# ChrisDud0257/GSASR

Hardware: AMD Instinct MI355X
Metric: HR Mpixels/sec fwd+bwd (x4, 1 Gaussian/LR px); achieved HBM GB/s vs roofline (higher is better)
Workload: dtype f32; 1 GPU; config2: 256x256 LR -> x4 (1024^2 HR), 65536 Gaussians, fwd+bwd; H=1024, W=1024, gaussians=65536, cutoff_k_box=336, launch=eager (faster than hipgraph replay: 67.6 vs 75.3 us/step), forward_subtile_px=8, parallelism=single

## Files before the change

### gsasr_amd/csrc/splat_common.h

```cpp
#ifndef GSASR_SPLAT_COMMON_H
#define GSASR_SPLAT_COMMON_H
#include <hip/hip_runtime.h>

#include <atomic>
#include <cmath>
#include <cstdint>
#include <cstdio>
#include <cstdlib>
#include <cstring>
#include <mutex>
#include <vector>

#include "gsasr_splat.h"

namespace gsasr_detail {

int fail(int code, const char *msg);
int hip_fail(hipError_t e, const char *where);
const char *last_error_message();
struct KernelChoice { unsigned flags; int list_cap; };
KernelChoice registered_choice(const gsasr_dims *d);
float default_cutoff();
void store_default_cutoff(float tau);

// ... 476 lines not shown
    if (cutoff != 0.f) return cutoff;
    const double tau = std::log((double)(s > 1 ? s : 1) / (double)GSASR_SPLAT_DEFAULT_EPS);
    return (float)(tau < 16.0 ? 16.0 : tau > (double)GSASR_SPLAT_EXACT_CUTOFF ? (double)GSASR_SPLAT_EXACT_CUTOFF : tau);
}

inline bool batch_uniform(const gsasr_dims *d, int &h, int &w)
{
    h = w = 0;
    if (d->batch <= 1) return false;
    for (int b = 1; b < d->batch; ++b)
        if (d->sample_hw[2 * b] != d->sample_hw[0] || d->sample_hw[2 * b + 1] != d->sample_hw[1]) return false;
    h = d->sample_hw[0];
    w = d->sample_hw[1];
    return true;
}

inline Params make_params(const gsasr_dims *d, const Layout &L, const gsasr_view *vw = nullptr)
{
    Params P;
    const gsasr_dims pd = policy_dims(d, vw);
    const bool bviews = vw && d->batch > 1;
    double scale_w = vw ? (double)vw->full_w : (double)d->w, scale_h = vw ? (double)vw->full_h : (double)d->h;
    double full_wmin = scale_w, full_hmin = scale_h;
    if (bviews) {
        for (int b = 1; b < d->batch; ++b) {
            scale_w = std::fmax(scale_w, (double)vw[b].full_w);
            scale_h = std::fmax(scale_h, (double)vw[b].full_h);
            full_wmin = std::fmin(full_wmin, (double)vw[b].full_w);
            full_hmin = std::fmin(full_hmin, (double)vw[b].full_h);
        }
    }
    P.s = d->s; P.h = d->h; P.w = d->w; P.row0 = d->row0; P.row1 = d->row1;
    P.bounded = d->dmax >= 0.f;
    P.dmax = P.bounded ? d->dmax : INFINITY;
    const float tau = resolve_cutoff(d->cutoff, d->s);
    P.kcut = tau > 0.f ? (float)(std::sqrt(2.0 * (double)tau) * (1.0 + 1e-6)) : 0.f;
    P.adapt_cells = P.adapt_cells4 = 0.f;
    P.adapt_ring = 0;
    P.count_words = (int)(L.count_bytes / 4);
    P.ext_groups = L.ext_groups;
    P.dead_off = (int)L.dead_off_words;
    {
        double wmin = full_wmin, hmin = full_hmin;
        if (d->batch > 1 && !bviews) {
            for (int b = 0; b < d->batch; ++b) {
                hmin = std::fmin(hmin, (double)d->sample_hw[2 * b]);
                wmin = std::fmin(wmin, (double)d->sample_hw[2 * b + 1]);
            }
        }
        P.cap_px_x = P.bounded ? (float)((double)d->dmax * 0.5 * (wmin - 1.0)) : INFINITY;
        P.cap_px_y = P.bounded ? (float)((double)d->dmax * 0.5 * (hmin - 1.0)) : INFINITY;
    }
    const bool adapt = ((d->cutoff == 0.f && default_cutoff() == 0.f) || (d->flags & GSASR_FLAG_CUTOFF_CAP)) && P.kcut > 0.f && adapt_env();
    P.adapt_ring = adapt && tau >= 16.f;
    static const bool gradtau_on = !(dev_switch("GSASR_SPLAT_GRADTAU") && atoi(dev_switch("GSASR_SPLAT_GRADTAU")) == 0);
    const bool whole = d->row0 == 0 && d->row1 == d->h && !vw;
    P.kb_max = (adapt && gradtau_on && whole) ? (float)(std::sqrt(2.0 * (double)GSASR_SPLAT_GRAD_TAU) * (1.0 + 1e-6)) : 0.f;
    if (P.bounded && adapt) {
        const int B = batch_of(d);
        const double dpx = (double)d->dmax * 0.5 * (scale_w - 1.0), dpy = (double)d->dmax * 0.5 * ((B > 1 && !bviews ? (double)d->slot : scale_h) - 1.0);
        const double half = (d->flags & GSASR_FLAG_CONTINUOUS) ? 1.0 : 0.0;
        const double mx = std::floor(dpx + 1.02) + half, my = std::floor(dpy + 1.02) + half;
        const double cx = std::ceil(2.0 * mx / (double)CELL) + 1.0, cy = std::ceil(2.0 * my / (double)CELL) + 1.0;
        const double cells = std::fmin(cx, (double)L.ncx) * std::fmin(cy, (double)L.ncy);
        P.adapt_cells = (float)std::fmin(cells, 1.0e9) * (1.f + 1e-6f);
        if ((double)d->s < 8.0 * (double)L.ncells && L.ncells + 1 + NDEAD > FUSED_CELLS_HOST) {
            const double bx = std::ceil(2.0 * mx / (4.0 * CELL)) + 1.0, by = std::ceil(2.0 * my / (4.0 * CELL)) + 1.0;
            P.adapt_cells4 = (float)std::fmin(std::fmin(bx, std::ceil(L.ncx / 4.0)) * std::fmin(by, std::ceil(L.ncy / 4.0)), 1.0e9) * (1.f + 1e-6f);
        }
    }
    P.ncx = L.ncx; P.ncy = L.ncy; P.ncells = L.ncells;
    P.flags = d->flags;
    constexpr unsigned BWD_ANY = GSASR_FLAG_BWD_GAUSSIAN | GSASR_FLAG_BWD_TILE | GSASR_FLAG_BWD_ATOMIC | GSASR_FLAG_BWD_HOME;
    if (!(P.flags & BWD_ANY))
        P.flags |= registered_choice(&pd).flags & (GSASR_FLAG_BWD_GAUSSIAN | GSASR_FLAG_BWD_TILE | GSASR_FLAG_BWD_HOME);
    if (!(P.flags & BWD_ANY))
        P.flags |= bwd_env() == 2 ? GSASR_FLAG_BWD_TILE : bwd_env() == 3 ? GSASR_FLAG_BWD_ATOMIC : bwd_env() == 4 ? GSASR_FLAG_BWD_HOME : 0u;
    P.batch = batch_of(d);
    P.slot = d->batch > 1 ? d->slot : d->h;
    P.nper = d->batch > 1 ? d->s / d->batch : d->s;
    P.part_k = L.part_k;
    P.bt_hlog = bt_tall(&pd) ? 5 : 4;
    batch_uniform(d, P.geo_h, P.geo_w);
    P.grad_rows = d->grad_rows > 0 ? d->grad_rows : P.slot;
    P.tl_hlog = L.tl_hlog; P.tl_cap = L.tl_cap; P.tl_ntx = L.tl_ntx; P.tl_ntiles = L.tl_ntiles;
    P.u8 = nullptr; P.u8_rows = P.u8_cols = 0; P.u8_swap = 0u; P.u8_pitch = 0;
    P.loss_target = nullptr; P.loss_grad = nullptr; P.loss_part = nullptr; P.loss_weight = P.loss_eps = 0.f;
    P.loss_kind = P.loss_sum = P.loss_trows = P.loss_nsx = 0;
    return P;
}

void note_plan(const void *ws, const gsasr_dims *d, size_t plan_bytes, int part_k, int tl_hlog, int tl_cap, const gsasr_view *vw = nullptr);
Layout plan_layout(const gsasr_dims *d, const void *ws, bool *noted = nullptr, const gsasr_view *vw = nullptr);
int check_ws(const gsasr_dims *dims, const void *ws, size_t ws_bytes, Layout &L, bool planning = false, const gsasr_view *vw = nullptr);

int u8_args_check(const gsasr_dims *dims, const unsigned char *out, int crop_rows, int crop_cols, size_t pitch, unsigned u8_flags);
int loss_args_check(const gsasr_dims *dims, const gsasr_loss *loss);

#define HIP_TRY(expr)                                    \
    do {                                                 \
        hipError_t _e = (expr);                          \
        if (_e != hipSuccess) return hip_fail(_e, #expr); \
    } while (0)

struct Box {
    int c0, c1, r0, r1;
    float ex, ey;
    int cls;
    bool near;
};

constexpr double WINDOW_EPS = 0.02;

template <bool VIEW = false>
__device__ __forceinline__ Box gaussian_box(float sx, float sy, float x, float y, const Params &P, const Geo &g, float kcut,
                                            const ViewArg &vw = ViewArg{0, 0, 0, 0, nullptr})
{
    Box b;
    float ext_x = P.dmax, ext_y = P.dmax;
    if (kcut > 0.f) {
        ext_x = fminf(ext_x, kcut * fabsf(sx));
        ext_y = fminf(ext_y, kcut * fabsf(sy));
    }
    const Scale sc = view_scale<VIEW>(vw, g);
    const double hx = 0.5 * (double)(sc.gw - 1), hy = 0.5 * (double)(sc.gh - 1);
    double cxp = ((double)x + 1.0) * hx, cyp = ((double)y + 1.0) * hy + (double)g.base;
    if (VIEW) { cxp -= (double)sc.ox; cyp -= (double)sc.oy; }
    const double ex = (double)ext_x * hx, ey = (double)ext_y * hy;
    b.ex = (float)ex;
    b.ey = (float)ey;
    const double pad = (P.flags & GSASR_FLAG_CONTINUOUS) ? 1.0 : 0.0;
    const double lox = ceil(cxp - ex - WINDOW_EPS) - pad, hix = floor(cxp + ex + WINDOW_EPS) + pad;
    const double loy = ceil(cyp - ey - WINDOW_EPS) - pad, hiy = floor(cyp + ey + WINDOW_EPS) + pad;
    const bool finite = (sx - sx == 0.f) && (sy - sy == 0.f) && (x - x == 0.f) && (y - y == 0.f);
    b.c0 = (int)fmax(lox, 0.0);
    b.c1 = (int)fmin(hix, (double)(g.w - 1));
    b.r0 = (int)fmax(loy, (double)max(P.row0, g.base));
    b.r1 = (int)fmin(hiy, (double)(min(P.row1, g.base + g.h) - 1));
    b.near = false;
    if (!finite || b.c0 > b.c1 || b.r0 > b.r1 || !(hix >= 0.0) || !(hiy >= (double)g.base)) {
        b.cls = 2;
        if (finite) {
            const double rmin = (double)max(P.row0, g.base), rmax = (double)(min(P.row1, g.base + g.h) - 1);
            const double dpx = (double)P.dmax * hx + 1.0, dpy = (double)P.dmax * hy + 1.0;
            b.near = !P.bounded || (cxp - dpx <= (double)(g.w - 1) && cxp + dpx >= 0.0 && cyp - dpy <= rmax && cyp + dpy >= rmin);
        }
    } else if (!(b.ex <= (float)RCAP_PX && b.ey <= (float)RCAP_PX))
        b.cls = 1;
    else
        b.cls = 0;
    return b;
}

template <int N>
__device__ __forceinline__ unsigned dpp_row_ror(unsigned v)
{
    return (unsigned)__builtin_amdgcn_update_dpp(0, (int)v, 0x120 + N, 0xf, 0xf, false);
}

__device__ __forceinline__ unsigned wave_max_u32(unsigned v)
{
    v = max(v, dpp_row_ror<1>(v));
    v = max(v, dpp_row_ror<2>(v));
    v = max(v, dpp_row_ror<4>(v));
    v = max(v, dpp_row_ror<8>(v));
    const unsigned a = (unsigned)__builtin_amdgcn_readlane((int)v, 0), b = (unsigned)__builtin_amdgcn_readlane((int)v, 16);
    const unsigned c = (unsigned)__builtin_amdgcn_readlane((int)v, 32), d = (unsigned)__builtin_amdgcn_readlane((int)v, 48);
    return max(max(a, b), max(c, d));
}

__device__ __forceinline__ unsigned wave_add_u32(unsigned v)
{
    v += dpp_row_ror<1>(v);
    v += dpp_row_ror<2>(v);
    v += dpp_row_ror<4>(v);
    v += dpp_row_ror<8>(v);
    return ((unsigned)__builtin_amdgcn_readlane((int)v, 0) + (unsigned)__builtin_amdgcn_readlane((int)v, 16)) +
           ((unsigned)__builtin_amdgcn_readlane((int)v, 32) + (unsigned)__builtin_amdgcn_readlane((int)v, 48));
}

__device__ __forceinline__ float wave_add_f32(float v)
{
    v += __builtin_bit_cast(float, dpp_row_ror<1>(__builtin_bit_cast(unsigned, v)));
    v += __builtin_bit_cast(float, dpp_row_ror<2>(__builtin_bit_cast(unsigned, v)));
    v += __builtin_bit_cast(float, dpp_row_ror<4>(__builtin_bit_cast(unsigned, v)));
    v += __builtin_bit_cast(float, dpp_row_ror<8>(__builtin_bit_cast(unsigned, v)));
    const int i = __builtin_bit_cast(int, v);
    return (__builtin_bit_cast(float, __builtin_amdgcn_readlane(i, 0)) + __builtin_bit_cast(float, __builtin_amdgcn_readlane(i, 16))) +
           (__builtin_bit_cast(float, __builtin_amdgcn_readlane(i, 32)) + __builtin_bit_cast(float, __builtin_amdgcn_readlane(i, 48)));
}

__device__ __forceinline__ float wave_sum(float v)
{
    for (int o = 32; o > 0; o >>= 1) v += __shfl_xor(v, o);
    return v;
}

__device__ __forceinline__ float adapt_kcut(const Params &P, unsigned maxcount, unsigned nlarge, unsigned nnear, unsigned ext_x,
                                            unsigned ext_y, float &tau, unsigned &K, unsigned maxblock = 0u)
{
    const float tau_cap = 0.5f * P.kcut * P.kcut;
    tau = tau_cap;
    K = 0u;
    if (!(P.adapt_cells > 0.f) && !P.adapt_ring) return P.kcut;
    float Kn = INFINITY;
    if (P.adapt_cells > 0.f) {
        Kn = (float)maxcount * P.adapt_cells;
        if (P.adapt_cells4 > 0.f) Kn = fminf(Kn, (float)maxblock * P.adapt_cells4);
    }
    float far_terms = (float)nnear;
    if (P.adapt_ring) {
        const float cx = fminf(ceilf((float)(2u * (min(ext_x, 130u) + 1u)) * (1.f / CELL)) + 1.f, (float)P.ncx);
        const float cy = fminf(ceilf((float)(2u * (min(ext_y, 130u) + 1u)) * (1.f / CELL)) + 1.f, (float)P.ncy);
        if ((float)maxcount * cx * cy < Kn) {
            Kn = (float)maxcount * cx * cy * (1.f + 1e-6f);
            far_terms += (float)maxcount * (2.1f * (cx + cy) + 5.f);
        }
    }
    const float Kf = fmaxf(Kn + (float)nlarge, 1.f);
    K = (unsigned)fminf(Kf, 4.0e9f);
    const float budget = GSASR_SPLAT_DEFAULT_EPS - far_terms * __builtin_amdgcn_exp2f(-tau_cap * 1.44269504f) * (1.f + 1e-5f);
    if (!(budget >= 0.25f * GSASR_SPLAT_DEFAULT_EPS)) return P.kcut;
    const float t = fmaxf(__log2f(Kf / budget) * 0.69314718f + 1e-3f, 16.f);
    if (!(t < tau_cap)) return P.kcut;
    tau = t;
    return fminf(sqrtf(2.f * t) * (1.f + 1e-6f), P.kcut);
}

__device__ __forceinline__ unsigned reach_of(unsigned ext, float kc, float kcut, float cap_px)
{
    if (ext < 2u || !(kc < kcut) || !((float)(ext - 2u) < cap_px - 1.f)) return ext;
    return min(ext, (unsigned)ceilf((float)(ext - 2u) * (kc / kcut) * (1.f + 1e-6f)) + 2u);
}

__device__ __forceinline__ unsigned count_index(int k, int ncells, int dead_off)
{
    return k <= ncells ? (unsigned)k : (unsigned)(dead_off + (k - ncells - 1) * 16);
}

struct BatchSizes {
    unsigned short h[GSASR_MAX_BATCH], w[GSASR_MAX_BATCH];
};
struct BatchViews {
    int4 v[GSASR_MAX_BATCH];
};

__device__ __forceinline__ float sigmoidf_(float v) { return 1.f / (1.f + expf(-v)); }

__device__ __forceinline__ void prologue_one(const float *__restrict__ q, float step, int h, int w, float (&o)[8])
{
#pragma clang fp contract(off)
    const float sx = 0.99999f * sigmoidf_(q[0]) + 1e-6f;
    const float sy = 0.99999f * sigmoidf_(q[1]) + 1e-6f;
    const float alpha = sigmoidf_(q[3]);
    const float W = (float)w, H = (float)h;
    const float iw1 = 1.f / (W - 1.f), ih1 = 1.f / (H - 1.f);
    o[0] = sy / step * 2.f * iw1;
    o[1] = sx / step * 2.f * ih1;
    o[2] = 0.999999f * tanhf(q[2]);
    const float c0 = q[7] * 2.f - 1.f, c1 = q[8] * 2.f - 1.f;
    o[3] = (c0 + 1.f - (float)(1.0 / (double)w)) * W * iw1 - 1.f;
    o[4] = (c1 + 1.f - (float)(1.0 / (double)h)) * H * ih1 - 1.f;
    o[5] = sigmoidf_(q[4]) * alpha;
    o[6] = sigmoidf_(q[5]) * alpha;
    o[7] = sigmoidf_(q[6]) * alpha;
}

struct StepSrc {
    const float *step;
    const float *sm;
    int stride;
    float def_step;
    int *mismatch;
    float *keep;
};

typedef float v2f __attribute__((ext_vector_type(2)));

enum StorePolicy { ST_PLAIN = 0, ST_WT = 1, ST_NT = 2 };
#ifndef GSASR_ST_IMAGE
#define GSASR_ST_IMAGE ST_WT
#endif
#ifndef GSASR_ST_IMAGE_CHW
#define GSASR_ST_IMAGE_CHW ST_PLAIN
#endif
#ifndef GSASR_ST_IMAGE_U8
#define GSASR_ST_IMAGE_U8 ST_PLAIN
#endif
#ifndef GSASR_ST_GRAD
#define GSASR_ST_GRAD ST_PLAIN
#endif
#ifndef GSASR_ST_PLAN
#define GSASR_ST_PLAN ST_PLAIN
#endif
constexpr StorePolicy ST_IMAGE = GSASR_ST_IMAGE;
constexpr StorePolicy ST_IMAGE_CHW = GSASR_ST_IMAGE_CHW;
constexpr StorePolicy ST_IMAGE_U8 = GSASR_ST_IMAGE_U8;
constexpr StorePolicy ST_GRAD = GSASR_ST_GRAD;
constexpr StorePolicy ST_PLAN = GSASR_ST_PLAN;

typedef float v4f __attribute__((ext_vector_type(4)));
typedef unsigned v2u __attribute__((ext_vector_type(2)));

template <StorePolicy POL>
__device__ __forceinline__ void store_out(float *p, float v)
{
// ... 332 lines not shown
```

### gsasr_amd/csrc/splat_plan.hip

```cpp
#include "splat_common.h"

using namespace gsasr_detail;

namespace {

__global__ __launch_bounds__(64) void k_batch_geo(BatchSizes S, int batch, int slot, int w, int4 *__restrict__ geo)
{
    const int b = threadIdx.x;
    if (b < batch) geo[b] = make_int4((int)S.h[b], (int)S.w[b], b * slot, b * w);
}

__global__ __launch_bounds__(64) void k_batch_views(BatchViews S, int batch, int4 *__restrict__ tab)
{
    const int b = threadIdx.x;
    if (b < batch) tab[b] = S.v[b];
}

template <bool PROLOGUE, bool VIEW>
__global__ __launch_bounds__(256) void k_classify(Params P, const float *__restrict__ sigmas,
                                                  const float *__restrict__ coords, PlanView V,
                                                  const float *__restrict__ raw, StepSrc SS,
                                                  float *__restrict__ o_sig, float *__restrict__ o_xy, float *__restrict__ o_col,
                                                  ViewArg VW)
{
// ... 228 lines not shown
    }
    unsigned run = inc - sum, total = 0;
    for (int k = 0; k < 16; ++k) {
        const unsigned p = part[k];
        run += k < wv ? p : 0u;
        total += p;
    }
#pragma unroll
    for (int k = 0; k < 4; ++k) {
        if (base + k < n) start[base + k] = run;
        run += c[k];
    }
    if (t == 0) tot[blockIdx.x] = total;

}

__global__ __launch_bounds__(1024) void k_scan_fix(Params P, int n, unsigned *__restrict__ start,
                                                   const unsigned *__restrict__ tot, int nchunks,
                                                   const unsigned *__restrict__ count, unsigned *__restrict__ hdr)
{
    __shared__ unsigned s_off;
    const int t = threadIdx.x;
    (void)P; (void)count; (void)hdr;
    if (t < 64) {
        unsigned v = 0;
        for (int k = t; k < (int)blockIdx.x; k += 64) v += tot[k];
        for (int o = 32; o > 0; o >>= 1) v += (unsigned)__shfl_xor((int)v, o);
        if (t == 0) s_off = v;
    }
    __syncthreads();
    const unsigned off = s_off;
    const int base = blockIdx.x * SCAN_CHUNK + t * 4;
#pragma unroll
    for (int k = 0; k < 4; ++k)
        if (base + k < n) start[base + k] += off;
    if ((int)blockIdx.x == nchunks - 1 && t == 0) start[n] = off + tot[blockIdx.x];
}

template <int HLOG>
__device__ __forceinline__ unsigned tl_mask8(int tx, int ty, const uint4 bb, const uint4 qs, int row0)
{
    const int c0 = (int)(bb.x & 0x7fffu), c1 = (int)(bb.x >> 16), r0 = (int)(bb.y & 0x7fffu), r1 = (int)(bb.y >> 16);
    const int q0 = (r0 - row0) >> 3, cu0 = c0 >> 3;
    constexpr int NQY = 1 << (HLOG - 3);
    unsigned mask = 0u;
#pragma unroll
    for (int qy = 0; qy < NQY; ++qy) {
        const int G = ty * NQY + qy, y0 = row0 + (G << 3);
        if (!(r0 <= y0 + 7 && r1 >= y0)) continue;
        const unsigned t = (unsigned)(G - q0) & 7u, sh = (t & 3u) * 8u;
        const unsigned l = ((t < 4u ? qs.x : qs.z) >> sh) & 0xffu, h = ((t < 4u ? qs.y : qs.w) >> sh) & 0xffu;
        if (l > h) continue;
        const int lo = cu0 + (int)l, hi = h == 255u ? (c1 >> 3) : cu0 + (int)h;
        const int a = max(lo - 4 * tx, 0), b = min(hi - 4 * tx, 3);
        if (a <= b) mask |= ((2u << b) - (1u << a)) << (4 * qy);
    }
    return mask;
}

template <int HLOG>
__device__ __forceinline__ unsigned tl_mask(int tx, int ty, const uint4 bb, const uint2 sp, int row0)
{
    const int c0 = (int)(bb.x & 0x7fffu), c1 = (int)(bb.x >> 16), r0 = (int)(bb.y & 0x7fffu), r1 = (int)(bb.y >> 16);
    const bool spans = (bb.y & 0x8000u) != 0u;
    const int wb0 = (r0 - row0) >> SUBY_SHIFT, cu0 = c0 >> SUBX_SHIFT;
    constexpr int NB = 1 << (HLOG - 4);
    unsigned mask = 0u;
#pragma unroll
    for (int bnd = 0; bnd < NB; ++bnd) {
        const int G = ty * NB + bnd;
        const int y0 = row0 + (G << SUBY_SHIFT);
        int lo = cu0, hi = c1 >> SUBX_SHIFT;
        bool any = r0 <= y0 + SUBY - 1 && r1 >= y0;
        if (spans) {
            const unsigned t = (unsigned)(G - wb0) & 7u, sh = (t & 3u) * 8u;
            const unsigned l = ((t < 4u ? bb.z : sp.x) >> sh) & 0xffu, h = ((t < 4u ? bb.w : sp.y) >> sh) & 0xffu;
            lo = cu0 + (int)l;
            hi = cu0 + (int)h;
            any = any && l <= h;
        }
        const int q0 = max(lo - 4 * tx, 0), q1 = min(hi - 4 * tx, 3);
        if (any && q0 <= q1) {
            const unsigned bits = (2u << q1) - (1u << q0);
            if (r0 <= y0 + 7) mask |= bits << (8 * bnd);
            if (r1 >= y0 + 8) mask |= bits << (8 * bnd + 4);
        }
    }
    return mask;
}

constexpr int TLB = 4;

template <int HLOG>
__device__ __forceinline__ void tl_emit(const Params &P, const PlanView &V, bool emit, unsigned j, const uint4 bb, const uint2 sp,
                                        const uint4 qs, bool fine8)
{
    const int lane = threadIdx.x & 63;
    const unsigned long long below = (1ull << lane) - 1ull;
    int nx = 0, ntile = 0, tX0 = 0, tY0 = 0;
    if (emit) {
        const int c0 = (int)(bb.x & 0x7fffu), c1 = (int)(bb.x >> 16), r0 = (int)(bb.y & 0x7fffu), r1 = (int)(bb.y >> 16);
        tX0 = c0 >> 5;
        nx = (c1 >> 5) - tX0 + 1;
        tY0 = (r0 - P.row0) >> HLOG;
        ntile = nx * (((r1 - P.row0) >> HLOG) - tY0 + 1);
    }
    const unsigned ex = j | ((bb.x & 0x8000u) << 16);
    const bool slots = P.part_k > 0 && P.tl_hlog == P.bt_hlog;
    const bool wide = !slots || ntile > P.part_k;
    int ix = 0, iy = 0;
    for (int base = 0; __ballot(base < ntile) != 0ull; base += TLB) {
        unsigned m[TLB], ti[TLB], pos[TLB];
        unsigned long long mine[TLB];
#pragma unroll
        for (int k = 0; k < TLB; ++k) {
            const bool v = base + k < ntile;
            m[k] = !v ? 0u : fine8 ? tl_mask8<HLOG>(tX0 + ix, tY0 + iy, bb, qs, P.row0) : tl_mask<HLOG>(tX0 + ix, tY0 + iy, bb, sp, P.row0);
            ti[k] = (unsigned)((tY0 + iy) * P.tl_ntx + tX0 + ix);
            if (v) {
                const unsigned slot = wide ? 0xffu : (unsigned)(base + k);
                if (m[k]) m[k] |= slot << 16;
                else if (!wide) {
                    float4 *o = reinterpret_cast<float4 *>(V.part + ((size_t)j * P.part_k + slot) * 8);
                    o[0] = make_float4(0.f, 0.f, 0.f, 0.f);
                    o[1] = make_float4(0.f, 0.f, 0.f, 0.f);
                }
            }
            if (v && ++ix == nx) { ix = 0; ++iy; }
            mine[k] = 0ull;
            unsigned long long todo = __ballot(m[k] != 0u);
            while (todo) {
                const unsigned t0 = (unsigned)__builtin_amdgcn_readlane((int)ti[k], __builtin_ctzll(todo));
                const unsigned long long same = __ballot(m[k] != 0u && ti[k] == t0);
                if (m[k] != 0u && ti[k] == t0) mine[k] = same;
                todo &= ~same;
            }
        }
#pragma unroll
        for (int k = 0; k < TLB; ++k) {
            pos[k] = 0u;
            if (mine[k] && lane == __builtin_ctzll(mine[k]))
                pos[k] = atomicAdd(&V.tl_cursor[(size_t)ti[k] * TL_STRIDE], (unsigned)__builtin_popcountll(mine[k]));
        }
#pragma unroll
        for (int k = 0; k < TLB; ++k) {
            const int leader = mine[k] ? __builtin_ctzll(mine[k]) : 0;
            const unsigned at = (unsigned)__shfl((int)pos[k], leader) + (unsigned)__builtin_popcountll(mine[k] & below);
            if (mine[k] && at < (unsigned)P.tl_cap) V.tl_entries[(size_t)ti[k] * (size_t)P.tl_cap + at] = make_uint2(ex, m[k]);
        }
    }
}

constexpr int FUSED_PER_THREAD = 17, FUSED_CELLS = 256 * FUSED_PER_THREAD;
constexpr int FUSED_GROUPS = 128;
static_assert(FUSED_CELLS == FUSED_CELLS_HOST, "make_params decides with FUSED_CELLS_HOST which plans run a scan kernel");

template <bool FUSED_SCAN, int TLH, bool VIEW>
__global__ __launch_bounds__(256) void k_bin(Params P, const float *__restrict__ sigmas,
                                             const float *__restrict__ coords,
                                             const float *__restrict__ colors, PlanView V, int nblk, ViewArg VW)
{
    __shared__ unsigned s_start[FUSED_SCAN ? FUSED_CELLS + 1 : 1];
    __shared__ unsigned s_part[FUSED_SCAN ? 256 : 1];
    const int i = blockIdx.x * blockDim.x + threadIdx.x;
    const bool valid = i < P.s;
    unsigned c[FUSED_SCAN ? FUSED_PER_THREAD : 1];
    const bool adapting = P.adapt_cells > 0.f || P.adapt_ring != 0;
    unsigned key = 0u, rnk = 0u;
    float sx = 0.f, sy = 0.f, rho = 0.f, x = 0.f, y = 0.f, col0 = 0.f, col1 = 0.f, col2 = 0.f;
    if (valid) {
        key = V.key[i];
        rnk = V.rank[i];
        const size_t i3 = (size_t)i * stride3(P), i2 = (size_t)i * stride2(P);
        sx = sigmas[i3 + 0]; sy = sigmas[i3 + 1]; rho = sigmas[i3 + 2];
        x = coords[i2 + 0]; y = coords[i2 + 1];
        col0 = colors[i3 + 0]; col1 = colors[i3 + 1]; col2 = colors[i3 + 2];
    }
    unsigned g_mc = 0u, g_mc2 = 0u, g_nn = 0u, nlarge = 0u;
    uint2 ga = make_uint2(0u, 0u), gb = ga;
    if constexpr (FUSED_SCAN) {
        static_assert(NDEAD - NDEAD_NEAR == 64, "one near-dead counter per lane");
        const int ln = (int)threadIdx.x & 63;
        ga = *reinterpret_cast<const uint2 *>(V.blockmax + 16 * min(ln, nblk - 1));
        gb = *reinterpret_cast<const uint2 *>(V.blockmax + 16 * min(ln + 64, nblk - 1));
        {
            const uint2 n2 = *reinterpret_cast<const uint2 *>(V.cell_count + P.dead_off + (NDEAD_NEAR + ln) * 16);
            g_nn = n2.x;
            g_mc = n2.y;
            g_mc2 = V.cell_count[P.dead_off + ln * 16 + 1];
        }
        nlarge = V.cell_count[P.ncells];
#pragma unroll
        for (int k = 0; k < FUSED_PER_THREAD; ++k) {
            const int q = min((int)threadIdx.x * FUSED_PER_THREAD + k, P.ncells + NDEAD);
            c[k] = V.cell_count[count_index(q, P.ncells, P.dead_off)];
        }
        __builtin_amdgcn_sched_barrier(0);
    }
    float4 recA = make_float4(0.f, 0.f, 0.f, 0.f), recB = recA, finA = recA, finB = recA;
    uint4 bb = make_uint4(0u, 0u, 0u, 0u), bc = bb;
    uint4 qs = make_uint4(0u, 0xffffffffu, 0u, 0xffffffffu);
    bool fine8 = false;
    bool large = false;
    unsigned fb_rx = 0u, fb_ry = 0u;
    float kc = P.kcut, kc_tau = 0.f;
    unsigned kc_K = 0u, kc_mc = 0u, kc_nn = 0u;
    if constexpr (FUSED_SCAN) {
        if (adapting) {
            kc_mc = wave_max_u32(max(g_mc, g_mc2));
            kc_nn = wave_add_u32(g_nn);
            const unsigned ext = wave_max_u32(max(ga.x, gb.x)), eyt = wave_max_u32(max(ga.y, gb.y));
            kc = adapt_kcut(P, kc_mc, nlarge, kc_nn, P.adapt_ring ? ext : 0u, P.adapt_ring ? eyt : 0u, kc_tau, kc_K);
        } else {
            kc_tau = 0.5f * P.kcut * P.kcut;
        }
    } else {
        const int ncls = P.ncells + 1 + NDEAD;
        kc = adapt_kcut(P, V.hdr[2], V.cell_start[P.ncells + 1] - V.cell_start[P.ncells],
                        V.cell_start[ncls] - V.cell_start[P.ncells + 1 + NDEAD_NEAR], V.hdr[0], V.hdr[1], kc_tau, kc_K, V.hdr[6]);
        if (i == 0) {
            V.hdr[3] = __float_as_uint(kc);
            V.hdr[4] = __float_as_uint(kc_tau);
            V.hdr[5] = kc_K;
            V.hdr[7] = V.cell_start[ncls] - V.cell_start[P.ncells + 1 + NDEAD_NEAR];
            atomicMax(&V.hdr[8], reach_of(V.hdr[0], kc, P.kcut, P.cap_px_x));
            atomicMax(&V.hdr[9], reach_of(V.hdr[1], kc, P.kcut, P.cap_px_y));
        }
    }
    if (valid) {
        const int smp = P.batch > 1 ? i / P.nper : 0;
        const Geo g = sample_geo(P, V, smp);
        const ViewArg vws = sample_view<VIEW>(VW, smp);
        const Scale sc = view_scale<VIEW>(vws, g);
        Box b = gaussian_box<VIEW>(sx, sy, x, y, P, g, kc, vws);
        float kw = kc;
        if (b.cls == 2 && key <= (unsigned)P.ncells && kc != P.kcut) {
            b = gaussian_box<VIEW>(sx, sy, x, y, P, g, P.kcut, vws);
            kw = P.kcut;
            if (key < (unsigned)P.ncells) {
                fb_rx = (unsigned)ceilf(b.ex) + 2u;
                fb_ry = (unsigned)ceilf(b.ey) + 2u;
            }
        }
        large = key == (unsigned)P.ncells;
        const double dr = rho, dsx = sx, dsy = sy;
        const double w1 = -0.5 / (1.0 - dr * dr);
        const double w2 = 1.0 / (dsx * dsx), w3 = 1.0 / (dsx * dsy), w4 = 1.0 / (dsy * dsy);
        const double cinv_d = -2.0 * w1, hl = 0.5 * LOG2E;
        const float IX = (float)(sqrt(hl) / dsx);
        const float IY = (float)(sqrt(hl * cinv_d) / dsy);
        const float NR = (float)(-dr * sqrt(cinv_d));
        (void)w2; (void)w3; (void)w4;
        recA = make_float4(x, y, IX, NR);
        recB = make_float4(IY, col0, col1, col2);
        finA = make_float4((float)(-2.0 * w1), (float)(1.0 - dr * dr), rho, (float)(1.0 / dsx));
        finB = make_float4((float)(1.0 / dsy), __uint_as_float((unsigned)g.pxo), __uint_as_float((unsigned)smp),
                           __uint_as_float((unsigned)i));
        const float hx = 0.5f * (float)(sc.gw - 1), hy = 0.5f * (float)(sc.gh - 1);
        const bool needs_test = P.bounded && !(kw > 0.f && kw * fabsf(sx) * hx + 1.f <= P.dmax * hx &&
                                               kw * fabsf(sy) * hy + 1.f <= P.dmax * hy);
        if (b.cls == 2) {
            bb = make_uint4(0x7fffu, 0x7fffu, 0u, 0u);
        } else {
            bb.x = (unsigned)b.c0 | (needs_test ? 0x8000u : 0u) | ((unsigned)b.c1 << 16);
            bb.y = (unsigned)b.r0 | ((unsigned)b.r1 << 16);
            bb.z = bb.w = 0u;
            const int ty0 = (b.r0 - P.row0) >> SUBY_SHIFT, ty1 = (b.r1 - P.row0) >> SUBY_SHIFT;
            if (kw > 0.f && ty1 - ty0 < 8 && (b.c1 >> SUBX_SHIFT) - (b.c0 >> SUBX_SHIFT) <= 255) {
                const float spx = sx * hx, spy = sy * hy;
                double cxp = ((double)x + 1.0) * (double)hx, cyp = ((double)y + 1.0) * (double)hy + (double)g.base;
                if (VIEW) { cxp -= (double)sc.ox; cyp -= (double)sc.oy; }
                const float tau = 0.5f * kw * kw;
                const float omr = (float)(1.0 - dr * dr);
                const float iq = 1.f / (omr * spx * spy);
                const float qa = 0.5f * iq * (spy / spx), qb = -rho * iq, qc = 0.5f * iq * (spx / spy);
                const float umax = fabsf(spx) * kw, vmax = fabsf(spy) * kw;
                const float vstar = -qb * umax / (2.f * qc);
                const float disc0 = 4.f * qa * tau, disc2 = 4.f * qa * qc - qb * qb, i2qa = 0.5f / qa;
                const float eps = (float)WINDOW_EPS;
                const int tx0 = b.c0 >> SUBX_SHIFT;
                auto spans = [&](int shift, int first, int nb, unsigned (&lo4)[2], unsigned (&hi4)[2]) {
                    lo4[0] = lo4[1] = 0x01010101u;
                    hi4[0] = hi4[1] = 0u;
                    for (int t = 0; t < 8 && __ballot(t < nb) != 0ull; ++t) {
                        if (t >= nb) continue;
                        unsigned lo = 1u, hi = 0u;
                        const float v0 = (float)((double)(P.row0 + ((first + t) << shift)) - cyp) - eps,
                                    v1 = v0 + (float)((1 << shift) - 1) + 2.f * eps;
                        if (v1 >= -vmax && v0 <= vmax) {
                            const float a0 = fmaxf(v0, -vmax), a1 = fminf(v1, vmax);
                            const float vr = fminf(fmaxf(vstar, a0), a1), vl = fminf(fmaxf(-vstar, a0), a1);
                            const float dr_ = disc0 - disc2 * vr * vr;
                            const float dl_ = disc0 - disc2 * vl * vl;
                            const float uhi = (-qb * vr + sqrtf(fmaxf(dr_, 0.f))) * i2qa;
                            const float ulo = (-qb * vl - sqrtf(fmaxf(dl_, 0.f))) * i2qa;
                            const int xl = max(b.c0, (int)fmax(ceil(cxp + (double)(ulo - eps)), -1.0));
                            const int xh = min(b.c1, (int)fmin(floor(cxp + (double)(uhi + eps)), 40000.0));
                            if (xl <= xh && !(umax != umax)) {
                                lo = (unsigned)min(255, (xl >> SUBX_SHIFT) - tx0);
                                hi = (unsigned)min(255, (xh >> SUBX_SHIFT) - tx0);
                            }
                        }
                        const unsigned sh = 8u * (unsigned)(t & 3), keep = ~(0xffu << sh);
                        if (t < 4) { lo4[0] = (lo4[0] & keep) | (lo << sh); hi4[0] = (hi4[0] & keep) | (hi << sh); }
                        else { lo4[1] = (lo4[1] & keep) | (lo << sh); hi4[1] = (hi4[1] & keep) | (hi << sh); }
                    }
                };
                unsigned lo4[2], hi4[2];
                spans(SUBY_SHIFT, ty0, ty1 - ty0 + 1, lo4, hi4);
                const int q0 = (b.r0 - P.row0) >> 3, q1 = (b.r1 - P.row0) >> 3;
                if (V.qspan && q1 - q0 < 8) {
                    unsigned l8[2], h8[2];
                    spans(3, q0, q1 - q0 + 1, l8, h8);
                    qs = make_uint4(l8[0], h8[0], l8[1], h8[1]);
                    fine8 = true;
                }
                bb.z = lo4[0]; bb.w = hi4[0];
                bc.x = lo4[1]; bc.y = hi4[1];
                bb.y |= 0x8000u;
            }
            {
                Box w = b;
                bool test_b = needs_test;
                if (P.kb_max > 0.f && kw > P.kb_max) {
                    const Box t = gaussian_box<VIEW>(sx, sy, x, y, P, g, P.kb_max, vws);
                    if (t.cls != 2) {
                        w = t;
                        test_b = P.bounded && !(P.kb_max * fabsf(sx) * hx + 1.f <= P.dmax * hx && P.kb_max * fabsf(sy) * hy + 1.f <= P.dmax * hy);
                    }
                }
                const int bwid = w.c1 - w.c0 + 1, nr = w.r1 - w.r0 + 1;
                const int rpt = bwid <= 16 ? 8 : (bwid <= BWD_LX21_MAX ? 6 : (bwid <= 32 ? 4 : 2));
                const int pad = (rpt - nr % rpt) % rpt;
                const int lo = max(P.row0, g.base), hi = min(P.row1, g.base + g.h) - 1;
                int r0p = w.r0, r1p = w.r1;
                if (r1p + pad <= hi) r1p += pad;
                else if (r0p - pad >= lo) r0p -= pad;
                bc.z = (unsigned)r0p | ((unsigned)r1p << 16);
                bc.w = (unsigned)w.c0 | (test_b ? 0x8000u : 0u) | ((unsigned)w.c1 << 16);
            }
        }
    }
    {
        if (__ballot(fb_rx != 0u) != 0ull) {
            const unsigned wx = wave_max_u32(fb_rx), wy = wave_max_u32(fb_ry);
            if ((threadIdx.x & 63) == 0) {
                atomicMax(&V.hdr[8], wx);
                atomicMax(&V.hdr[9], wy);
            }
        }
    }
    if constexpr (FUSED_SCAN) {
        const int t = threadIdx.x, ncls = P.ncells + 1 + NDEAD;
        const int b0 = t * FUSED_PER_THREAD;
        unsigned sum = 0;
#pragma unroll
        for (int k = 0; k < FUSED_PER_THREAD; ++k) c[k] = b0 + k < ncls ? c[k] : 0u;
#pragma unroll
        for (int k = 0; k < FUSED_PER_THREAD; ++k) sum += c[k];
        unsigned inc = sum;
        for (int o = 1; o < 64; o <<= 1) {
            const unsigned v = (unsigned)__shfl_up((int)inc, o);
            if ((t & 63) >= o) inc += v;
        }
        if ((t & 63) == 63) s_part[t >> 6] = inc;
        __syncthreads();
        unsigned run = inc - sum;
        for (int k = 0; k < (t >> 6); ++k) run += s_part[k];
#pragma unroll
        for (int k = 0; k < FUSED_PER_THREAD; ++k) {
            if (b0 + k <= ncls) s_start[b0 + k] = run;
            run += c[k];
        }
        __syncthreads();
        if (blockIdx.x == 0) {
            for (int k = t; k <= ncls; k += 256) V.cell_start[k] = s_start[k];
            unsigned mx = 0, my = 0;
            for (int k = t; k < nblk; k += 256) {
                mx = max(mx, V.blockmax[16 * k + 0]);
                my = max(my, V.blockmax[16 * k + 1]);
            }
            mx = wave_max_u32(mx);
            my = wave_max_u32(my);
            __syncthreads();
            if ((t & 63) == 0) { s_part[t >> 6] = mx; s_part[4 + (t >> 6)] = my; }
            __syncthreads();
            if (t == 0) {
                const unsigned ex0 = max(max(s_part[0], s_part[1]), max(s_part[2], s_part[3]));
                const unsigned ey0 = max(max(s_part[4], s_part[5]), max(s_part[6], s_part[7]));
                V.hdr[0] = ex0;
                V.hdr[1] = ey0;
                atomicMax(&V.hdr[8], reach_of(ex0, kc, P.kcut, P.cap_px_x));
                atomicMax(&V.hdr[9], reach_of(ey0, kc, P.kcut, P.cap_px_y));
                V.hdr[2] = kc_mc;
                V.hdr[3] = __float_as_uint(kc);
                V.hdr[4] = __float_as_uint(kc_tau);
                V.hdr[5] = kc_K;
                V.hdr[7] = kc_nn;
            }
        }
    }
    if (!valid && TLH == 0) return;
    const unsigned j = valid ? (FUSED_SCAN ? s_start[key] : V.cell_start[key]) + rnk : 0u;
    if (valid) {
    const bool live = key <= (unsigned)P.ncells;
    const bool backward_records = !(P.flags & GSASR_FLAG_FORWARD_ONLY);
    if (live) {
        store_out<ST_PLAN>(V.rec + 2 * j + 0, recA);
        store_out<ST_PLAN>(V.rec + 2 * j + 1, recB);
        store_out<ST_PLAN>(V.bbox + 2 * j + 1, bc);
        if (V.qspan) V.qspan[j] = qs;
    }
    if (backward_records) {
        if (live) store_out<ST_PLAN>(V.fin + 2 * j + 0, finA);
        store_out<ST_PLAN>(V.fin + 2 * j + 1, finB);
    }
    store_out<ST_PLAN>(V.bbox + 2 * j, bb);
    store_out<ST_PLAN>(V.win + j, make_uint2(bb.x, bb.y));
    if (backward_records && live && (large || V.qspan || (P.flags & GSASR_FLAG_BWD_ATOMIC))) {
        reinterpret_cast<float4 *>(V.sums)[2 * (size_t)j] = make_float4(0.f, 0.f, 0.f, 0.f);
        reinterpret_cast<float4 *>(V.sums)[2 * (size_t)j + 1] = make_float4(0.f, 0.f, 0.f, 0.f);
        if (large) V.done[j] = 0u;
    }
    }
    if constexpr (TLH != 0)
        tl_emit<TLH == 0 ? 4 : TLH>(P, V, valid && key < (unsigned)P.ncells, j, bb, make_uint2(bc.x, bc.y), qs, fine8);
}

}

namespace gsasr_detail {

int launch_batch_geo(const gsasr_dims *dims, const PlanView &V, hipStream_t st)
{
    if (dims->batch <= 1) return GSASR_OK;
    int uh, uw;
    if (batch_uniform(dims, uh, uw)) return GSASR_OK;
    BatchSizes S;
    for (int b = 0; b < GSASR_MAX_BATCH; ++b) {
        S.h[b] = (unsigned short)(b < dims->batch ? dims->sample_hw[2 * b] : 0);
        S.w[b] = (unsigned short)(b < dims->batch ? dims->sample_hw[2 * b + 1] : 0);
    }
    hipLaunchKernelGGL(k_batch_geo, dim3(1), dim3(64), 0, st, S, dims->batch, dims->slot, dims->w, V.geo);
    HIP_TRY(hipGetLastError());
    return GSASR_OK;
}

int plan_impl(const float *sigmas, const float *coords, const float *colors, const gsasr_dims *dims, void *workspace,
              size_t workspace_bytes, void *stream, const float *raw, const StepSrc &SS, const gsasr_view *vw)
{
    Layout L;
    if (int rc = check_ws(dims, workspace, workspace_bytes, L, true, vw)) return rc;
    note_plan(workspace, dims, L.total, L.part_k, L.tl_hlog, L.tl_cap, vw);
    if (dims->s > 0 && (!sigmas || !coords || !colors)) return fail(GSASR_ERR_ARG, "null input pointer");
    hipStream_t st = (hipStream_t)stream;
    const Params P = make_params(dims, L, vw);
    const PlanView V = make_view(L, workspace, dims->flags);
    const ViewArg VW = view_arg(vw, dims->batch, (const char *)workspace + L.off_vtab);
    if (vw && dims->batch > 1) {
        BatchViews S;
        for (int b = 0; b < GSASR_MAX_BATCH; ++b)
            S.v[b] = b < dims->batch ? make_int4(vw[b].full_h, vw[b].full_w, vw[b].y0, vw[b].x0) : make_int4(0, 0, 0, 0);
        hipLaunchKernelGGL(k_batch_views, dim3(1), dim3(64), 0, st, S, dims->batch, (int4 *)((char *)workspace + L.off_vtab));
    }
    if (!(dims->flags & GSASR_FLAG_COUNTERS_CLEAN)) HIP_TRY(hipMemsetAsync(V.cell_count, 0, L.count_bytes, st));
    if (!raw)
        if (int rc = launch_batch_geo(dims, V, st)) return rc;
    const int nblk = classify_blocks(dims);
#define GSASR_CLASSIFY(ISVIEW) do { \
    if (raw) \
        hipLaunchKernelGGL((k_classify<true, ISVIEW>), dim3(nblk), dim3(256), 0, st, P, sigmas, coords, V, raw, SS, \
                           const_cast<float *>(sigmas), const_cast<float *>(coords), const_cast<float *>(colors), VW); \
    else \
        hipLaunchKernelGGL((k_classify<false, ISVIEW>), dim3(nblk), dim3(256), 0, st, P, sigmas, coords, V, (const float *)nullptr, \
                           SS, (float *)nullptr, (float *)nullptr, (float *)nullptr, VW); } while (0)
    if (vw) GSASR_CLASSIFY(true);
    else GSASR_CLASSIFY(false);
#undef GSASR_CLASSIFY
    const int ncls = L.ncells + 1 + NDEAD;
    const unsigned nbin = (unsigned)((dims->s + 255) / 256);
    static const int fused_max_blocks = dev_switch("GSASR_SPLAT_FUSED_MAX") ? atoi(dev_switch("GSASR_SPLAT_FUSED_MAX")) : FUSED_MAX_BLOCKS;
    if (ncls <= FUSED_CELLS && dims->s > 0 && (int)nbin <= fused_max_blocks && L.ext_groups <= FUSED_GROUPS) {
#define GSASR_BIN_V(F, ISVIEW) do { \
        const int tlh = P.tl_hlog; \
        if (tlh == 5) hipLaunchKernelGGL((k_bin<F, 5, ISVIEW>), dim3(nbin), dim3(256), 0, st, P, sigmas, coords, colors, V, L.ext_groups, VW); \
        else if (tlh == 4) hipLaunchKernelGGL((k_bin<F, 4, ISVIEW>), dim3(nbin), dim3(256), 0, st, P, sigmas, coords, colors, V, L.ext_groups, VW); \
        else hipLaunchKernelGGL((k_bin<F, 0, ISVIEW>), dim3(nbin), dim3(256), 0, st, P, sigmas, coords, colors, V, L.ext_groups, VW); } while (0)
#define GSASR_BIN(F) do { if (vw) GSASR_BIN_V(F, true); else GSASR_BIN_V(F, false); } while (0)
        GSASR_BIN(true);
    } else {
        if (ncls <= 2 * SCAN_CHUNK) {
            hipLaunchKernelGGL(k_scan, dim3(1), dim3(1024), 0, st, P, ncls, V.cell_count, V.cell_start, L.ext_groups, V.blockmax,
                               V.hdr);
        } else {
            const int nchunks = (ncls + SCAN_CHUNK - 1) / SCAN_CHUNK;
            hipLaunchKernelGGL(k_scan_local, dim3(nchunks), dim3(1024), 0, st, L.ncells, ncls, V.cell_count, V.cell_start,
                               V.scan_tot, L.ext_groups, V.blockmax, V.hdr, L.ncx, L.ncy, (int)(P.adapt_cells4 > 0.f), P.dead_off);
            hipLaunchKernelGGL(k_scan_fix, dim3(nchunks), dim3(1024), 0, st, P, ncls, V.cell_start, V.scan_tot, nchunks,
                               V.cell_count, V.hdr);
        }
        if (dims->s > 0) GSASR_BIN(false);
#undef GSASR_BIN
#undef GSASR_BIN_V
    }
    HIP_TRY(hipGetLastError());
    return GSASR_OK;
}

}

extern "C" {

int gsasr_splat_plan(const float *sigmas, const float *coords, const float *colors, const gsasr_dims *dims,
                     void *workspace, size_t workspace_bytes, void *stream)
{
    return plan_impl(sigmas, coords, colors, dims, workspace, workspace_bytes, stream, nullptr, StepSrc{});
}

int gsasr_splat_plan_view(const float *sigmas, const float *coords, const float *colors, const gsasr_dims *dims,
                          const gsasr_view *view, void *workspace, size_t workspace_bytes, void *stream)
{
    return plan_impl(sigmas, coords, colors, dims, workspace, workspace_bytes, stream, nullptr, StepSrc{}, norm_view(dims, view));
}

}
```

Baseline: 17920 HR Mpixels/s.

## Offload Gaussian constant math in fused k_bin to extra helper wavefronts

In the fused-scan variant, k_bin now launches twice as many threads. The extra 256 threads compute the double-precision Gaussian constants (IX, NR, IY, inverse covariance terms, inverse sigmas) into shared memory, while the original threads do the cell-count scan, so the FP64 math overlaps with the scan instead of running in series. The per-Gaussian input loads are also made unconditional with a clamped index and fenced by a sched_barrier, so they issue early. The helper threads must hit exactly as many __syncthreads as the main path (hardcoded, with extra barriers for block 0), which is fragile. The larger block also raises register and LDS pressure and may reduce occupancy.

```diff
diff --git a/gsasr_amd/csrc/splat_common.h b/gsasr_amd/csrc/splat_common.h
--- a/gsasr_amd/csrc/splat_common.h
+++ b/gsasr_amd/csrc/splat_common.h
@@ -652,6 +652,28 @@
     return b;
 }
 
+struct GaussConst {
+    float IX, NR, IY;
+    float c, kappa, isx, isy;
+};
+__device__ __forceinline__ GaussConst gaussian_const(float sx, float sy, float rho)
+{
+#pragma clang fp contract(off)
+    const double dr = rho, dsx = sx, dsy = sy;
+    const double omr = fma(-dr, dr, 1.0);
+    const double w1 = -0.5 / omr;
+    const double cinv_d = -2.0 * w1, hl = 0.5 * LOG2E;
+    GaussConst k;
+    k.IX = (float)(sqrt(hl) / dsx);
+    k.IY = (float)(sqrt(hl * cinv_d) / dsy);
+    k.NR = (float)(-dr * sqrt(cinv_d));
+    k.c = (float)cinv_d;
+    k.kappa = (float)omr;
+    k.isx = (float)(1.0 / dsx);
+    k.isy = (float)(1.0 / dsy);
+    return k;
+}
+
 template <int N>
 __device__ __forceinline__ unsigned dpp_row_ror(unsigned v)
 {
diff --git a/gsasr_amd/csrc/splat_plan.hip b/gsasr_amd/csrc/splat_plan.hip
--- a/gsasr_amd/csrc/splat_plan.hip
+++ b/gsasr_amd/csrc/splat_plan.hip
@@ -404,29 +404,46 @@
 }
 
 constexpr int FUSED_PER_THREAD = 17, FUSED_CELLS = 256 * FUSED_PER_THREAD;
+constexpr int BIN_THREADS = 256;
 constexpr int FUSED_GROUPS = 128;
 static_assert(FUSED_CELLS == FUSED_CELLS_HOST, "make_params decides with FUSED_CELLS_HOST which plans run a scan kernel");
 
 template <bool FUSED_SCAN, int TLH, bool VIEW>
-__global__ __launch_bounds__(256) void k_bin(Params P, const float *__restrict__ sigmas,
-                                             const float *__restrict__ coords,
-                                             const float *__restrict__ colors, PlanView V, int nblk, ViewArg VW)
+__global__ __launch_bounds__(FUSED_SCAN ? 2 * BIN_THREADS : BIN_THREADS) void k_bin(Params P, const float *__restrict__ sigmas,
+                                                         const float *__restrict__ coords,
+                                                         const float *__restrict__ colors, PlanView V, int nblk, ViewArg VW)
 {
     __shared__ unsigned s_start[FUSED_SCAN ? FUSED_CELLS + 1 : 1];
     __shared__ unsigned s_part[FUSED_SCAN ? 256 : 1];
-    const int i = blockIdx.x * blockDim.x + threadIdx.x;
+    __shared__ float s_const[FUSED_SCAN ? 7 : 1][FUSED_SCAN ? BIN_THREADS : 1];
+    const int i = blockIdx.x * BIN_THREADS + (threadIdx.x & (BIN_THREADS - 1));
+    if (FUSED_SCAN && threadIdx.x >= BIN_THREADS) {
+        if (i < P.s) {
+            const size_t i3 = (size_t)i * stride3(P);
+            const GaussConst k = gaussian_const(sigmas[i3 + 0], sigmas[i3 + 1], sigmas[i3 + 2]);
+            const int t = threadIdx.x - BIN_THREADS;
+            s_const[0][t] = k.IX; s_const[1][t] = k.NR; s_const[2][t] = k.IY; s_const[3][t] = k.c;
+            s_const[4][t] = k.kappa; s_const[5][t] = k.isx; s_const[6][t] = k.isy;
+        }
+        __syncthreads();
+        __syncthreads();
+        if (blockIdx.x == 0) { __syncthreads(); __syncthreads(); }
+        return;
+    }
     const bool valid = i < P.s;
     unsigned c[FUSED_SCAN ? FUSED_PER_THREAD : 1];
     const bool adapting = P.adapt_cells > 0.f || P.adapt_ring != 0;
     unsigned key = 0u, rnk = 0u;
     float sx = 0.f, sy = 0.f, rho = 0.f, x = 0.f, y = 0.f, col0 = 0.f, col1 = 0.f, col2 = 0.f;
-    if (valid) {
-        key = V.key[i];
-        rnk = V.rank[i];
-        const size_t i3 = (size_t)i * stride3(P), i2 = (size_t)i * stride2(P);
+    {
+        const int il = min(i, P.s - 1);
+        key = V.key[il];
+        rnk = V.rank[il];
+        const size_t i3 = (size_t)il * stride3(P), i2 = (size_t)il * stride2(P);
         sx = sigmas[i3 + 0]; sy = sigmas[i3 + 1]; rho = sigmas[i3 + 2];
         x = coords[i2 + 0]; y = coords[i2 + 1];
         col0 = colors[i3 + 0]; col1 = colors[i3 + 1]; col2 = colors[i3 + 2];
+        __builtin_amdgcn_sched_barrier(0);
     }
     unsigned g_mc = 0u, g_mc2 = 0u, g_nn = 0u, nlarge = 0u;
     uint2 ga = make_uint2(0u, 0u), gb = ga;
@@ -449,7 +466,8 @@
         }
         __builtin_amdgcn_sched_barrier(0);
     }
-    float4 recA = make_float4(0.f, 0.f, 0.f, 0.f), recB = recA, finA = recA, finB = recA;
+    unsigned fin_pxo = 0u, fin_smp = 0u;
+    GaussConst gk = {0.f, 0.f, 0.f, 0.f, 0.f, 0.f, 0.f};
     uint4 bb = make_uint4(0u, 0u, 0u, 0u), bc = bb;
     uint4 qs = make_uint4(0u, 0xffffffffu, 0u, 0xffffffffu);
     bool fine8 = false;
@@ -495,19 +513,10 @@
             }
         }
         large = key == (unsigned)P.ncells;
-        const double dr = rho, dsx = sx, dsy = sy;
-        const double w1 = -0.5 / (1.0 - dr * dr);
-        const double w2 = 1.0 / (dsx * dsx), w3 = 1.0 / (dsx * dsy), w4 = 1.0 / (dsy * dsy);
-        const double cinv_d = -2.0 * w1, hl = 0.5 * LOG2E;
-        const float IX = (float)(sqrt(hl) / dsx);
-        const float IY = (float)(sqrt(hl * cinv_d) / dsy);
-        const float NR = (float)(-dr * sqrt(cinv_d));
-        (void)w2; (void)w3; (void)w4;
-        recA = make_float4(x, y, IX, NR);
-        recB = make_float4(IY, col0, col1, col2);
-        finA = make_float4((float)(-2.0 * w1), (float)(1.0 - dr * dr), rho, (float)(1.0 / dsx));
-        finB = make_float4((float)(1.0 / dsy), __uint_as_float((unsigned)g.pxo), __uint_as_float((unsigned)smp),
-                           __uint_as_float((unsigned)i));
+        const double dr = rho;
+        if constexpr (!FUSED_SCAN) gk = gaussian_const(sx, sy, rho);
+        fin_pxo = (unsigned)g.pxo;
+        fin_smp = (unsigned)smp;
         const float hx = 0.5f * (float)(sc.gw - 1), hy = 0.5f * (float)(sc.gh - 1);
         const bool needs_test = P.bounded && !(kw > 0.f && kw * fabsf(sx) * hx + 1.f <= P.dmax * hx &&
                                                kw * fabsf(sy) * hy + 1.f <= P.dmax * hy);
@@ -657,6 +666,13 @@
     if (valid) {
     const bool live = key <= (unsigned)P.ncells;
     const bool backward_records = !(P.flags & GSASR_FLAG_FORWARD_ONLY);
+    const int tc = (int)threadIdx.x;
+    if constexpr (FUSED_SCAN)
+        gk = GaussConst{s_const[0][tc], s_const[1][tc], s_const[2][tc], s_const[3][tc], s_const[4][tc], s_const[5][tc], s_const[6][tc]};
+    const float4 recA = make_float4(x, y, gk.IX, gk.NR);
+    const float4 recB = make_float4(gk.IY, col0, col1, col2);
+    const float4 finA = make_float4(gk.c, gk.kappa, rho, gk.isx);
+    const float4 finB = make_float4(gk.isy, __uint_as_float(fin_pxo), __uint_as_float(fin_smp), __uint_as_float((unsigned)i));
     if (live) {
         store_out<ST_PLAN>(V.rec + 2 * j + 0, recA);
         store_out<ST_PLAN>(V.rec + 2 * j + 1, recB);
@@ -734,10 +750,10 @@
     static const int fused_max_blocks = dev_switch("GSASR_SPLAT_FUSED_MAX") ? atoi(dev_switch("GSASR_SPLAT_FUSED_MAX")) : FUSED_MAX_BLOCKS;
     if (ncls <= FUSED_CELLS && dims->s > 0 && (int)nbin <= fused_max_blocks && L.ext_groups <= FUSED_GROUPS) {
 #define GSASR_BIN_V(F, ISVIEW) do { \
-        const int tlh = P.tl_hlog; \
-        if (tlh == 5) hipLaunchKernelGGL((k_bin<F, 5, ISVIEW>), dim3(nbin), dim3(256), 0, st, P, sigmas, coords, colors, V, L.ext_groups, VW); \
-        else if (tlh == 4) hipLaunchKernelGGL((k_bin<F, 4, ISVIEW>), dim3(nbin), dim3(256), 0, st, P, sigmas, coords, colors, V, L.ext_groups, VW); \
-        else hipLaunchKernelGGL((k_bin<F, 0, ISVIEW>), dim3(nbin), dim3(256), 0, st, P, sigmas, coords, colors, V, L.ext_groups, VW); } while (0)
+        const int tlh = P.tl_hlog, nthr = (F) ? 2 * BIN_THREADS : BIN_THREADS; \
+        if (tlh == 5) hipLaunchKernelGGL((k_bin<F, 5, ISVIEW>), dim3(nbin), dim3(nthr), 0, st, P, sigmas, coords, colors, V, L.ext_groups, VW); \
+        else if (tlh == 4) hipLaunchKernelGGL((k_bin<F, 4, ISVIEW>), dim3(nbin), dim3(nthr), 0, st, P, sigmas, coords, colors, V, L.ext_groups, VW); \
+        else hipLaunchKernelGGL((k_bin<F, 0, ISVIEW>), dim3(nbin), dim3(nthr), 0, st, P, sigmas, coords, colors, V, L.ext_groups, VW); } while (0)
 #define GSASR_BIN(F) do { if (vw) GSASR_BIN_V(F, true); else GSASR_BIN_V(F, false); } while (0)
         GSASR_BIN(true);
     } else {
```

After: 17970 HR Mpixels/s, median of 6. About the same (+0.3%).
